# mazpie/genrl

Hardware: AMD Instinct MI355X
Metric: world-model+imag update steps/sec (B32xL32x64x64x3) (higher is better)
Workload: dtype f32 (storage, accumulation, every non-GEMM kernel and the fp32-MFMA GEMMs; the forward / dgrad / weight-gradient products of the imagination rollout, of the Dense+LN+SiLU chains from 192 rows up and of the encoder / decoder convolutions take fp32 operands pre-split into two fp16 planes of the scaled

## Files before the change

genrl_amd/csrc/dist.hip:

```cpp
#include "common.h"
#include <math.h>

namespace {

template <int W>
struct Cat {
  float p, pn, s;
  __device__ __forceinline__ void init(float logit, bool valid, int K, float a) {
    const float l = valid ? logit : -INFINITY;
    const float m = group_max<W>(l);
    const float e = valid ? expf(l - m) : 0.f;
    const float z = group_sum<W>(e);
    p = e / z;
    const float u = valid ? a * p + (1.0f - a) / K : 0.f;
    s = group_sum<W>(u);
    pn = u / s;
  }
  __device__ __forceinline__ float backward(float g, bool valid, float a) const {
    const float gi = valid ? g : 0.f;
    const float dot = group_sum<W>(gi * pn);
    const float du = (gi - dot) / s;
    const float dp = a * du;
    const float dot2 = group_sum<W>(valid ? dp * p : 0.f);
    return valid ? p * (dp - dot2) : 0.f;
// ... 119 lines not shown
  const float logit = sum + (bias ? bias[n0 + k] : 0.f);
  Cat<32> cat;
  cat.init(logit, valid, 32, a);
  const long g = (long)min(orow, M - 1) * S + lat;
  const float score = valid ? (q ? cat.pn / q[g * 32 + k] : cat.pn) : -INFINITY;
  const int best = group_argmax<32>(score, k);
  if (valid) {
    C[(long)orow * ldc + n0 + k] = logit;
    sample[g * 32 + k] = (k == best) ? 1.0f : 0.0f;
    const float sc2 = (sample2 || idx2) ? (scale2 ? scale2[orow] : 1.0f) : 1.0f;
    if (sample2) sample2[g * 32 + k] = (k == best) ? sc2 : 0.0f;
    if (idx2 && k == 0) idx2[g] = sc2 != 0.0f ? best : -1;
  }
}

template <int W>
__global__ __launch_bounds__(1024) void onehot_bwd_kernel(const float* __restrict__ logits,
                                                          const float* __restrict__ gsample,
                                                          float* __restrict__ dlogits, long G, int K, float a,
                                                          int accumulate, PlaneOut xo, int rowlen, MaskedGrad mg) {
  __shared__ float redm[16];
  const long g = ((long)blockIdx.x * blockDim.x + threadIdx.x) / W;
  const int k = threadIdx.x % W;
  const bool valid = (g < G) && (k < K);
  const long gi = g < G ? g : G - 1;
  const float l = valid ? logits[gi * K + k] : 0.f;
  Cat<W> c;
  c.init(l, valid, K, a);
  float gs = (valid && gsample) ? gsample[gi * K + k] : 0.f;
  if (valid && mg.g2) gs += (mg.scale ? mg.scale[gi / mg.S] : 1.0f) * mg.g2[gi * K + k];
  const float d = c.backward(gs, valid, a);
  float o = 0.f;
  if (valid) {
    o = accumulate ? dlogits[gi * K + k] + d : d;
    if (dlogits) dlogits[gi * K + k] = o;
  }
  if (xo.p) {
    const float am = wave_max(fabsf(o));
    if ((threadIdx.x & 63) == 0) redm[threadIdx.x >> 6] = am;
    __syncthreads();
    float m = redm[0];
    for (int w = 1; w < (int)(blockDim.x >> 6); ++w) m = fmaxf(m, redm[w]);
    const float inv = h2_inv_of(m);
    if (valid) h2_store1(xo, (long)blockIdx.x * xo.ld + threadIdx.x, o, h2_scale_of(inv));
    if (threadIdx.x == 0) xo.inv[blockIdx.x] = inv;
  }
}

template <int W>
__global__ __launch_bounds__(256) void cat_kl_fwd_kernel(const float* __restrict__ lp, const float* __restrict__ lq,
                                                         float* __restrict__ kl, float* __restrict__ ent_p,
                                                         float* __restrict__ ent_q, int S, int K, float a) {
  __shared__ float red[16];
  const long row = blockIdx.x;
  constexpr int GPB = 256 / W;
  const int k = threadIdx.x % W, gsub = threadIdx.x / W;
  float akl = 0.f, aep = 0.f, aeq = 0.f;
  for (int s0 = 0; s0 < S; s0 += GPB) {
    const int s = s0 + gsub;
// ... 35 lines not shown
  const float lpp = clamp_log(cp.pn), lqq = clamp_log(cq.pn);
  if (dlp) {
    const float d = cp.backward(valid ? (lpp - lqq + 1.0f) : 0.f, valid, a);
    if (valid) dlp[gi * K + k] = gp[row] * d;
  }
  if (dlq) {
    const float d = cq.backward(valid ? (-cp.pn / cq.pn) : 0.f, valid, a);
    if (valid) dlq[gi * K + k] = gq[row] * d;
  }
}

struct TwoHot {
  int below, above;
  float wb, wa;
};
__device__ __forceinline__ TwoHot twohot_target(const float* __restrict__ buckets, float x, int lane) {
  const float xs = symlogf_(x);
  int le = 0, gt = 0;
  for (int j = lane; j < 255; j += 64) {
    le += (buckets[j] <= xs);
    gt += (buckets[j] > xs);
  }
  le = (int)wave_sum((float)le);
  gt = (int)wave_sum((float)gt);
  TwoHot t;
  t.below = min(max(le - 1, 0), 254);
  t.above = min(max(255 - gt, 0), 254);
  const bool eq = t.below == t.above;
  const float db = eq ? 1.0f : fabsf(buckets[t.below] - xs);
  const float da = eq ? 1.0f : fabsf(buckets[t.above] - xs);
  const float tot = db + da;
  t.wb = da / tot;
  t.wa = db / tot;
  return t;
}

__global__ __launch_bounds__(256) void twohot_fwd_kernel(const float* __restrict__ logits,
                                                         const float* __restrict__ x,
                                                         const float* __restrict__ buckets, float* __restrict__ out,
                                                         long R, int mode, long ld) {
  const int lane = threadIdx.x & 63;
  const long row = (long)blockIdx.x * 4 + (threadIdx.x >> 6);
  if (row >= R) return;
  const float* lr = logits + row * ld;
  float m = -INFINITY;
  for (int j = lane; j < 255; j += 64) m = fmaxf(m, lr[j]);
  m = wave_max(m);
  float z = 0.f, sb = 0.f;
  for (int j = lane; j < 255; j += 64) {
    const float e = expf(lr[j] - m);
    z += e;
    sb += e * buckets[j];
  }
  z = wave_sum(z);
  if (mode == 1) {
    sb = wave_sum(sb);
    if (lane == 0) out[row] = symexpf_(sb / z);
    return;
  }
  const float lse = m + logf(z);
  const TwoHot t = twohot_target(buckets, x[row], lane);
  if (lane == 0) out[row] = t.wb * (lr[t.below] - lse) + t.wa * (lr[t.above] - lse);
}

__global__ __launch_bounds__(256) void twohot_bwd_kernel(const float* __restrict__ logits,
                                                         const float* __restrict__ x,
                                                         const float* __restrict__ buckets,
                                                         const float* __restrict__ gout, float* __restrict__ dlogits,
                                                         long R, int mode, long ld, long ldd) {
  const int lane = threadIdx.x & 63;
  const long row = (long)blockIdx.x * 4 + (threadIdx.x >> 6);
  if (row >= R) return;
  const float* lr = logits + row * ld;
  float m = -INFINITY;
  for (int j = lane; j < 255; j += 64) m = fmaxf(m, lr[j]);
  m = wave_max(m);
  float z = 0.f, sb = 0.f;
  for (int j = lane; j < 255; j += 64) {
    const float e = expf(lr[j] - m);
    z += e;
    sb += e * buckets[j];
  }
  z = wave_sum(z);
  sb = wave_sum(sb);
  const float g = gout[row];
  float* dr = dlogits + row * ldd;
  if (ldd > 255 && lane == 63) dr[255] = 0.f;
  if (mode == 1) {
    const float mu = sb / z;
    const float ds = g * expf(fabsf(mu));
    for (int j = lane; j < 255; j += 64) dr[j] = ds * (expf(lr[j] - m) / z) * (buckets[j] - mu);
    return;
  }
  const TwoHot t = twohot_target(buckets, x[row], lane);
  for (int j = lane; j < 255; j += 64) {
    float tg = 0.f;
    if (j == t.below) tg += t.wb;
    if (j == t.above) tg += t.wa;
    dr[j] = g * (tg - expf(lr[j] - m) / z);
  }
}

__global__ __launch_bounds__(256) void kl_balance_fwd_kernel(const float* __restrict__ kl, long R, float mix, float free_,
                                                            float* __restrict__ loss) {
  __shared__ float red[8];
  float a = 0.f;
  for (long i = threadIdx.x; i < R; i += 256) a += fmaxf(kl[i], free_);
  a = block_sum_256(a, red);
  if (threadIdx.x == 0) {
    const float m = a / (float)R;
    *loss = mix * m + (1.0f - mix) * m;
  }
}
__global__ void kl_balance_bwd_kernel(const float* __restrict__ kl, const float* __restrict__ gloss, long R, float mix,
// ... 42 lines not shown
  for (int i = threadIdx.x; i < E; i += 256) {
    const float d = mp[i] - ((float)op[i] / 255.0f - 0.5f);
    a += d * d;
  }
  a = block_sum_256(a, red);
  if (threadIdx.x == 0) like[n] = -a;
}
__global__ void mse_bwd_kernel(const float* __restrict__ mean, const uint8_t* __restrict__ obs,
                               const float* __restrict__ glike, float* __restrict__ dmean, long total, int E) {
  const long i = (long)blockIdx.x * blockDim.x + threadIdx.x;
  if (i >= total) return;
  const float d = mean[i] - ((float)obs[i] / 255.0f - 0.5f);
  dmean[i] = -2.0f * d * glike[i / E];
}

__global__ __launch_bounds__(256) void maxcos_fwd_kernel(const float* __restrict__ u, const float* __restrict__ v,
                                                         const long* __restrict__ urow, float* __restrict__ out,
                                                         long R, int E) {
  const int lane = threadIdx.x & 63;
  const long row = (long)blockIdx.x * 4 + (threadIdx.x >> 6);
  if (row >= R) return;
  const float* ur = u + (urow ? urow[row] : row) * E;
  const float* vr = v + row * E;
  float su = 0.f, sv = 0.f;
  for (int j = lane; j < E; j += 64) {
    su += ur[j] * ur[j];
    sv += vr[j] * vr[j];
  }
  const float mn = fmaxf(sqrtf(wave_sum(su)), sqrtf(wave_sum(sv)));
  float d = 0.f;
  for (int j = lane; j < E; j += 64) d += (ur[j] / mn) * (vr[j] / mn);
  d = wave_sum(d);
  if (lane == 0) out[row] = d;
}
__global__ __launch_bounds__(256) void maxcos_bwd_kernel(const float* __restrict__ u, const float* __restrict__ v,
                                                         const long* __restrict__ urow, const float* __restrict__ gout,
                                                         float* __restrict__ dv, long R, int E) {
  const int lane = threadIdx.x & 63;
  const long row = (long)blockIdx.x * 4 + (threadIdx.x >> 6);
  if (row >= R) return;
  const float* ur = u + (urow ? urow[row] : row) * E;
  const float* vr = v + row * E;
  float su = 0.f, sv = 0.f, uv = 0.f;
  for (int j = lane; j < E; j += 64) {
    su += ur[j] * ur[j];
    sv += vr[j] * vr[j];
    uv += ur[j] * vr[j];
  }
  su = wave_sum(su);
  sv = wave_sum(sv);
  uv = wave_sum(uv);
  const float g = gout[row];
  float* dr = dv + row * E;
  const float wv = sv > su ? 1.0f : (sv == su ? 0.5f : 0.0f);
  for (int j = lane; j < E; j += 64) dr[j] = g * (ur[j] / fmaxf(su, sv) - wv * 2.0f * uv * vr[j] / (sv * sv));
}

constexpr int AL_MAX_T = 32, AL_MAX_NF = 8, AL_MAX_D = AL_MAX_NF * (AL_MAX_T - AL_MAX_NF);
template <int EPT>
__global__ __launch_bounds__(256) void align_index_kernel(const float* __restrict__ ct, const float* __restrict__ ca,
                                                          long* __restrict__ urow, int T, long N, int E, int nf) {
  constexpr int AL_SLOTS = AL_MAX_D + AL_MAX_T + AL_MAX_NF;
  __shared__ float swave[4][AL_SLOTS];
  __shared__ float sdot[AL_SLOTS];
  __shared__ int sbest;
  const long n = blockIdx.x;
  const int W = T - nf;
  const int nd = nf * W, ntot = nd + T + nf;
  const int wv = threadIdx.x >> 6;
  const int lane = threadIdx.x & 63;
  float cj[AL_MAX_NF][EPT > 0 ? EPT : 1];
  if (EPT > 0) {
#pragma unroll
    for (int j = 0; j < AL_MAX_NF; ++j)
#pragma unroll
      for (int i = 0; i < EPT; ++i) {
        const int e = threadIdx.x + i * 256;
        cj[j][i] = (j < nf && e < E) ? ct[((long)j * N + n) * E + e] : 0.f;
      }
  }
  for (int tau = 0; tau < T; ++tau) {
    const float* vr = ca + ((long)tau * N + n) * E;
    float vv = 0.f;
    float d[AL_MAX_NF];
#pragma unroll
    for (int j = 0; j < AL_MAX_NF; ++j) d[j] = 0.f;
    if (EPT > 0) {
#pragma unroll
      for (int i = 0; i < EPT; ++i) {
        const int e = threadIdx.x + i * 256;
        const float v = e < E ? vr[e] : 0.f;
        vv += v * v;
#pragma unroll
        for (int j = 0; j < AL_MAX_NF; ++j) d[j] += v * cj[j][i];
      }
    } else {
      for (int e = threadIdx.x; e < E; e += 256) {
        const float v = vr[e];
        vv += v * v;
#pragma unroll
        for (int j = 0; j < AL_MAX_NF; ++j)
          if (j < nf) d[j] += v * ct[((long)j * N + n) * E + e];
      }
    }
    vv = wave_sum(vv);
    if (lane == 0) swave[wv][nd + tau] = vv;
#pragma unroll
    for (int j = 0; j < AL_MAX_NF; ++j) {
      if (j < nf) {
        const int t = tau - j;
        const float s = wave_sum(d[j]);
        if (lane == 0 && t >= 0 && t < W) swave[wv][t * nf + j] = s;
      }
    }
  }
  for (int j = 0; j < nf; ++j) {
    const float* ur = ct + ((long)j * N + n) * E;
    float uu = 0.f;
    if (EPT > 0) {
#pragma unroll
      for (int i = 0; i < EPT; ++i) {
        float c = 0.f;
#pragma unroll
        for (int jj = 0; jj < AL_MAX_NF; ++jj)
          if (jj == j) c = cj[jj][i];
        uu += c * c;
      }
// ... 64 lines not shown
int genrl_onehot_bwd_planes_only_ok(int K, int rowlen) {
  return (K == 4 || K == 8 || K == 16 || K == 32 || K == 64) && rowlen > 0 && rowlen % 64 == 0 && rowlen <= 1024 && rowlen % K == 0;
}

static int onehot_bwd_impl(const float* logits, const float* gsample, float* dlogits, long G, int K, float unimix,
                     int accumulate, PlaneOut xo, int rowlen, void* stream, MaskedGrad mg = MaskedGrad{nullptr, nullptr, 1}) {
  GENRL_ENTER();
  if (G <= 0) return GENRL_OK;
  if ((!gsample && !mg.g2) || (mg.g2 && mg.S <= 0)) return GENRL_EINVAL;
  if (xo.p && (rowlen <= 0 || xo.ld < rowlen || !xo.inv || rowlen % K || (G * K) % rowlen)) return GENRL_EINVAL;
  if (K > MAX_K) return GENRL_EINVAL;
  return dispatch_w(K, [&](auto w) {
    constexpr int W = decltype(w)::value;
    const bool rowblk = xo.p && genrl_onehot_bwd_planes_only_ok(K, rowlen);
    if (!dlogits && (accumulate || !rowblk)) return (int)GENRL_EINVAL;
    if (rowblk)
      hipLaunchKernelGGL((onehot_bwd_kernel<W>), dim3((G * K) / rowlen), dim3(rowlen), 0, (hipStream_t)stream, logits,
                         gsample, dlogits, G, K, unimix, accumulate, xo, rowlen, mg);
    else
      hipLaunchKernelGGL((onehot_bwd_kernel<W>), dim3(cdiv(G * W, 256)), dim3(256), 0, (hipStream_t)stream, logits,
                         gsample, dlogits, G, K, unimix, accumulate, PlaneOut{nullptr, 0, 0, nullptr}, rowlen, mg);
    GENRL_CHECK_LAUNCH();
    if (xo.p && !rowblk)
      return genrl_split_h2(dlogits, rowlen, (int)((G * K) / rowlen), rowlen, xo.p, xo.ld, xo.plane, xo.inv, 0, stream);
    return GENRL_OK;
  });
}
int genrl_onehot_bwd(const float* logits, const float* gsample, float* dlogits, long G, int K, float unimix,
                     int accumulate, void* stream) {
  return onehot_bwd_impl(logits, gsample, dlogits, G, K, unimix, accumulate, PlaneOut{nullptr, 0, 0, nullptr}, 1, stream);
}
int genrl_onehot_bwd_h2(const float* logits, const float* gsample, float* dlogits, long G, int K, float unimix,
                        int accumulate, uint16_t* dp, int rowlen, long ldp, long plane, float* inv, void* stream) {
  return onehot_bwd_impl(logits, gsample, dlogits, G, K, unimix, accumulate, PlaneOut{dp, ldp, plane, inv}, rowlen, stream);
}
// ... 73 lines not shown
  GENRL_CHECK_LAUNCH();
  return GENRL_OK;
}

int genrl_twohot_fwd(const float* logits, long ld, const float* x, const float* buckets, float* out, long R, int mode,
                     void* stream) {
  GENRL_ENTER();
  if (R <= 0) return GENRL_OK;
  if (ld < 255) return GENRL_EINVAL;
  hipLaunchKernelGGL(twohot_fwd_kernel, dim3(cdiv(R, 4)), dim3(256), 0, (hipStream_t)stream, logits, x, buckets, out, R,
                     mode, ld);
  GENRL_CHECK_LAUNCH();
  return GENRL_OK;
}

int genrl_twohot_bwd(const float* logits, long ld, const float* x, const float* buckets, const float* gout,
                     float* dlogits, long ldd, long R, int mode, void* stream) {
  GENRL_ENTER();
  if (R <= 0) return GENRL_OK;
  if (ld < 255 || ldd < 255) return GENRL_EINVAL;
  hipLaunchKernelGGL(twohot_bwd_kernel, dim3(cdiv(R, 4)), dim3(256), 0, (hipStream_t)stream, logits, x, buckets, gout,
                     dlogits, R, mode, ld, ldd);
  GENRL_CHECK_LAUNCH();
  return GENRL_OK;
}

int genrl_lambda_return_fwd(const float* reward, const float* value, float* ret, int H, long N, float disc, float lam,
                            void* stream) {
  GENRL_ENTER();
  if (N <= 0) return GENRL_OK;
  hipLaunchKernelGGL(lambda_return_fwd_kernel, dim3(cdiv(N, 256)), dim3(256), 0, (hipStream_t)stream, reward, value,
                     ret, H, N, disc, lam);
  GENRL_CHECK_LAUNCH();
  return GENRL_OK;
}

int genrl_lambda_return_bwd(const float* gret, float* dreward, float* dvalue, int H, long N, float disc, float lam,
                            int zero_tail, void* stream) {
  GENRL_ENTER();
// ... 14 lines not shown

int genrl_mse_bwd(const float* mean, const uint8_t* obs, const float* glike, float* dmean, long Nimg, int E,
                  void* stream) {
  GENRL_ENTER();
  const long total = Nimg * E;
  if (total <= 0) return GENRL_OK;
  hipLaunchKernelGGL(mse_bwd_kernel, dim3(cdiv(total, 256)), dim3(256), 0, (hipStream_t)stream, mean, obs, glike, dmean,
                     total, E);
  GENRL_CHECK_LAUNCH();
  return GENRL_OK;
}

int genrl_maxcos_fwd(const float* u, const float* v, const long* urow, float* out, long R, int E, void* stream) {
  GENRL_ENTER();
  if (R <= 0) return GENRL_OK;
  hipLaunchKernelGGL(maxcos_fwd_kernel, dim3(cdiv(R, 4)), dim3(256), 0, (hipStream_t)stream, u, v, urow, out, R, E);
  GENRL_CHECK_LAUNCH();
  return GENRL_OK;
}

int genrl_maxcos_bwd(const float* u, const float* v, const long* urow, const float* gout, float* dv, long R, int E,
                     void* stream) {
  GENRL_ENTER();
  if (R <= 0) return GENRL_OK;
  hipLaunchKernelGGL(maxcos_bwd_kernel, dim3(cdiv(R, 4)), dim3(256), 0, (hipStream_t)stream, u, v, urow, gout, dv, R,
                     E);
  GENRL_CHECK_LAUNCH();
  return GENRL_OK;
}

int genrl_align_index(const float* ct, const float* ca, long* urow, int T, long N, int E, int nf, void* stream) {
  GENRL_ENTER();
  if (N <= 0) return GENRL_OK;
  if (T > AL_MAX_T || nf > AL_MAX_NF || nf >= T) return GENRL_EINVAL;
#define GO(EPTV) hipLaunchKernelGGL((align_index_kernel<EPTV>), dim3(N), dim3(256), 0, (hipStream_t)stream, ct, ca, urow, T, N, E, nf)
  if (E <= 512) GO(2); else if (E <= 1024) GO(4); else if (E <= 1536) GO(6); else if (E <= 2048) GO(8); else GO(0);
#undef GO
  GENRL_CHECK_LAUNCH();
  return GENRL_OK;
}

// ... 2 lines not shown
```

genrl_amd/csrc/stats.hip:

```cpp
#include "actor_heads.h"
#include <algorithm>
#include <math.h>

namespace {

constexpr int NT = 1024;

__global__ __launch_bounds__(NT) void moments_kernel(const float* __restrict__ x, long n, float* __restrict__ out) {
  __shared__ double red[16];
  double s = 0.0, q = 0.0, a = 0.0;
  for (long i = threadIdx.x; i < n; i += NT) {
    const double v = x[i];
    s += v; q += v * v; a += fabs(v);
  }
  s = block_sum_d(s, red); q = block_sum_d(q, red); a = block_sum_d(a, red);
  if (threadIdx.x == 0) {
    const double mean = s / n;
    const double var = n > 1 ? fmax((q - n * mean * mean) / (n - 1), 0.0) : NAN;
    out[0] = (float)mean; out[1] = (float)sqrt(var); out[2] = (float)(a / n); out[3] = (float)(q / n);
  }
}

__device__ __forceinline__ unsigned key_of(float f) {
  const unsigned u = __builtin_bit_cast(unsigned, f);
  return (u & 0x80000000u) ? ~u : (u | 0x80000000u);
}
__device__ __forceinline__ float val_of(unsigned k) {
  const unsigned u = (k & 0x80000000u) ? (k & 0x7FFFFFFFu) : ~k;
  return __builtin_bit_cast(float, u);
}

__global__ __launch_bounds__(NT) void quantile_ema_kernel(const float* __restrict__ x, long n, float q0, float q1,
                                                           float alpha, float* __restrict__ ema,
                                                           float* __restrict__ out ) {
  __shared__ unsigned hist[4][256];
  __shared__ unsigned prefix[4];
  __shared__ long rank[4];
  __shared__ float wgt[2];
  __shared__ int slot[4], nslot;
  if (threadIdx.x == 0) {
    const float r0 = q0 * (float)(n - 1), r1 = q1 * (float)(n - 1);
    rank[0] = (long)floorf(r0); rank[1] = (long)ceilf(r0); rank[2] = (long)floorf(r1); rank[3] = (long)ceilf(r1);
    wgt[0] = r0 - floorf(r0); wgt[1] = r1 - floorf(r1);
    for (int s = 0; s < 4; ++s) prefix[s] = 0u;
  }
  constexpr int KPT = 16;
  const bool inreg = n <= (long)KPT * NT;
  unsigned keys[KPT];
  if (inreg) {
#pragma unroll
    for (int j = 0; j < KPT; ++j) {
      const long i = (long)j * NT + threadIdx.x;
      keys[j] = i < n ? key_of(x[i]) : 0u;
    }
  }
  for (int round = 0; round < 4; ++round) {
    const int shift = 24 - 8 * round;
    for (int i = threadIdx.x; i < 4 * 256; i += NT) (&hist[0][0])[i] = 0u;
    if (threadIdx.x == 0) {
      int ns = 0;
      for (int s2 = 0; s2 < 4; ++s2) {
        int found = -1;
        for (int t = 0; t < s2; ++t)
          if (prefix[t] == prefix[s2]) { found = slot[t]; break; }
        slot[s2] = found >= 0 ? found : ns++;
      }
      nslot = ns;
    }
    __syncthreads();
    const unsigned mask = round == 0 ? 0u : (0xFFFFFFFFu << (shift + 8));
    unsigned pf[4];
    const int ns = nslot;
#pragma unroll
    for (int h = 0; h < 4; ++h) pf[h] = 0xFFFFFFFFu;
#pragma unroll
    for (int s2 = 3; s2 >= 0; --s2) pf[slot[s2]] = prefix[s2];
    auto count = [&](unsigned k) {
#pragma unroll
      for (int h = 0; h < 4; ++h)
        if (h < ns && (k & mask) == pf[h]) atomicAdd(&hist[h][(k >> shift) & 255u], 1u);
    };
    if (inreg) {
#pragma unroll
      for (int j = 0; j < KPT; ++j)
        if ((long)j * NT + threadIdx.x < n) count(keys[j]);
    } else {
      for (long i = threadIdx.x; i < n; i += NT) count(key_of(x[i]));
    }
    __syncthreads();
    if (threadIdx.x < 4) {
      const int s2 = threadIdx.x, h = slot[s2];
      long r = rank[s2];
      int b = 0;
      for (; b < 255; ++b) {
        const unsigned c = hist[h][b];
        if (r < (long)c) break;
        r -= c;
      }
      rank[s2] = r;
      prefix[s2] |= ((unsigned)b) << shift;
    }
    __syncthreads();
  }
  if (threadIdx.x == 0) {
    const float v[4] = {val_of(prefix[0]), val_of(prefix[1]), val_of(prefix[2]), val_of(prefix[3])};
    float qv[2];
#pragma unroll
    for (int j = 0; j < 2; ++j) {
      const float a = v[2 * j], b = v[2 * j + 1], w = wgt[j];
      qv[j] = w < 0.5f ? a + w * (b - a) : b - (b - a) * (1.0f - w);
    }
    const float e0 = alpha * qv[0] + (1.0f - alpha) * ema[0], e1 = alpha * qv[1] + (1.0f - alpha) * ema[1];
    ema[0] = e0; ema[1] = e1;
    out[0] = e0; out[1] = fmaxf(e1 - e0, 1.0f); out[2] = qv[0]; out[3] = qv[1];
  }
// ... 231 lines not shown
```

genrl_amd/ops.py:

```python
import os
import ctypes
import torch
from torch.autograd import Function

from ._lib import lib, check, GenrlHipError, struct as _cstruct

UNIMIX = 0.99
gemm_profile = None


from .streams import raw_current_stream as _stream
from .streams import timed_start, timed_end


def _p(t):
    if t is None:
        return None
    if not t.is_cuda:
        raise GenrlHipError('genrl_amd ops need tensors on the MI355X (no CPU fallback)')
    assert t.is_contiguous(), 'non-contiguous tensor handed to a HIP op'
    return t.data_ptr()


_PREF = _cstruct('genrl_planes_ref')
# ... 519 lines not shown
        v = t.reshape(R, 255).contiguous()
    return v, (v.stride(0) if R > 1 else 255)


class _TwoHot(Function):
    @staticmethod
    def forward(ctx, logits, x, mode):
        lg, ld = _rows255(_f32(logits))
        R = lg.shape[0]
        b = twohot_buckets(lg.device)
        xx = x.reshape(R).contiguous() if x is not None else None
        out = torch.empty(R, device=lg.device)
        check(lib().genrl_twohot_fwd(_prows(lg), ld, _p(xx), _p(b), _p(out), R, mode, _stream()), 'twohot_fwd')
        ctx.save_for_backward(lg, xx if xx is not None else lg.new_empty(0))
        ctx.mode, ctx.ld, ctx.lshape = mode, ld, logits.shape
        return out.reshape(logits.shape[:-1])

    @staticmethod
    def backward(ctx, g):
        lg, xx = ctx.saved_tensors
        R = lg.shape[0]
        d = torch.empty(R, 256, device=lg.device)
        check(lib().genrl_twohot_bwd(_prows(lg), ctx.ld, _p(xx) if ctx.mode == 0 else None, _p(twohot_buckets(lg.device)),
                                     _p(g.reshape(R).contiguous()), _p(d), 256, R, ctx.mode, _stream()), 'twohot_bwd')
        return d[:, :255].view(ctx.lshape), None, None


def twohot_logprob(logits, x):
    return _TwoHot.apply(logits, x.detach(), 0)


def twohot_mean(logits):
    return _TwoHot.apply(logits, None, 1).unsqueeze(-1)



class _LambdaReturn(Function):
    @staticmethod
    def forward(ctx, reward, value, disc, lam):
        Hv = value.shape[0]
# ... 1912 lines not shown
```

genrl_amd/ops_planes.py:

```python
import os

import torch
from torch.autograd import Function

from ._lib import lib, check, struct as _cstruct
from . import planes
from . import planes as pl
from . import ops
from .ops import _p, _f32, _ln_param_targets, _wgrad_target, _bias_grad, sgemm, fill, UNIMIX

_stream = ops._stream


def _ln_fwd(pre_ptr, gamma, beta, y_ptr, mean_ptr, rstd_ptr, M, N, eps, P, row0):
    check(lib().genrl_ln_act_fwd_h2(pre_ptr, N, _p(gamma), _p(beta), y_ptr, N, mean_ptr, rstd_ptr, M, N, eps, 1,
                                    P.ptr(row0), P.ld, P.plane, P.inv_ptr(row0), _stream()), 'ln_act_fwd_h2')


def _ln_bwd(dy_ptr, pre_ptr, gamma, beta, mean_ptr, rstd_ptr, dpre_ptr, M, N, P, row0, g0=None, g1=None, g2=None, ws=None,
            acc_p=0):
    check(lib().genrl_ln_act_bwd_h2(dy_ptr, N, pre_ptr, N, _p(gamma), _p(beta), mean_ptr, rstd_ptr, dpre_ptr, N, _p(g0),
                                    _p(g1), _p(g2), _p(ws), M, N, 1, acc_p, P.ptr(row0), P.ld, P.plane, P.inv_ptr(row0),
                                    _stream()), 'ln_act_bwd_h2')

# ... 308 lines not shown
class _LinearPlanes(Function):
    @staticmethod
    def forward(ctx, x, W, b, P, r0):
        x2 = _f32(x).reshape(-1, x.shape[-1]).contiguous()
        M, K = x2.shape
        N = W.shape[0]
        if P is None:
            P, r0 = planes.split(x2), 0
        Np = (N + 3) // 4 * 4
        y = torch.empty(M, Np, device=x.device)
        planes.gemm(P, planes.weight(W), y, Np, b, M, N, a_row0=r0)
        ctx.save_for_backward(x2, W)
        ctx.bias = b
        ctx.xshape = x.shape
        ctx.in_planes = (P, r0) if (ctx.needs_input_grad[1] and planes.tn_ok(M, N, K, K) and r0 % 4 == 0) else None
        return (y if Np == N else y[:, :N]).view(*x.shape[:-1], N)

    @staticmethod
    def backward(ctx, dy):
        x2, W = ctx.saved_tensors
        M, K = x2.shape
        N = W.shape[0]
        b = ctx.bias
        dy2, ldy = ops._rows_ld(dy.reshape(M, N))
        dx = dW = db = None
        tn = ctx.needs_input_grad[1] and ctx.in_planes is not None and planes.tn_ok(M, N, K, K)
        dyp = planes.split(dy2) if (ctx.needs_input_grad[0] or tn) else None
        if ctx.needs_input_grad[0]:
            dx = torch.empty(M, K, device=dy.device)
            planes.gemm(dyp, planes.weight(W, transpose=True), dx, K, None, M, K)
            dx = dx.reshape(ctx.xshape)
        if ctx.needs_input_grad[1]:
            tgt, acc, dW = _wgrad_target(W)
            if tn:
                planes.gemm_tn(dyp, ctx.in_planes[0], tgt, K, N, K, M, accumulate=acc, b_row0=ctx.in_planes[1])
            else:
                sgemm(dy2, 1, ldy, x2, 1, K, tgt, K, None, N, K, M, accumulate=acc)
        if b is not None and ctx.needs_input_grad[2]:
            db = _bias_grad(b, dy2, ldy)
        return dx, dW, db, None, None


# ... 428 lines not shown
```

include/genrl_hip.h:

```cpp
#ifndef GENRL_HIP_H
#define GENRL_HIP_H
#include <stdint.h>
#ifdef __cplusplus
extern "C" {
#endif

long genrl_sgemm_ws_floats(int M, int N, int K);
int genrl_set_gemm_precision(int mode);
int genrl_sgemm_last_pipe(void);
int genrl_gemm_precision(void);
int genrl_sgemm(const float* A, long a_rs, long a_ks, const float* B, long b_rs, long b_ks, float* C, long ldc,
                const float* bias, int M, int N, int K, int accumulate, float* ws, long ws_floats, void* stream);

int genrl_sgemm_conv(const float* A, long a_rs, long a_ks, const float* B, long b_rs, long b_ks, float* C, long ldc,
                     const float* bias, int M, int N, int K, int accumulate, float* ws, long ws_floats, int which,
                     int img_h, int img_w, int img_c, int ksize, void* stream);

int genrl_split_h2(const float* x, long ldx, int R, int Cn, uint16_t* out, long ld_out, long plane, float* inv, int transpose,
                   void* stream);
int genrl_gemm_h2(const uint16_t* a0, long a0_ld, long a0_plane, const float* a0_inv, const uint16_t* b0, long b0_ld, long b0_plane,
                  const float* b0_inv, int k0, const uint16_t* a1, long a1_ld, long a1_plane, const float* a1_inv,
                  const uint16_t* b1, long b1_ld, long b1_plane, const float* b1_inv, int k1,
                  float* C, long ldc, const float* bias, int M, int N, int accumulate, void* stream);
int genrl_gemm_h2_pair(const uint16_t* a, long a_ld, long a_plane, const float* a_inv, int k,
// ... 245 lines not shown
int genrl_onehot_bwd_masked(const float* logits, const float* gsample, const float* g2, const float* scale2, int S, float* dlogits,
                            long G, int K, float unimix, int accumulate, void* stream);
int genrl_cat_kl_fwd(const float* lp, const float* lq, float* kl, float* ent_p, float* ent_q, long R, int S, int K,
                     float unimix, void* stream);
int genrl_cat_kl_bwd(const float* lp, const float* lq, const float* gp, const float* gq, float* dlp, float* dlq, long R,
                     int S, int K, float unimix, void* stream);

int genrl_kl_balance_fwd(const float* kl, long R, float mix, float free_nats, float* loss, void* stream);
int genrl_kl_balance_bwd(const float* kl, const float* gloss, long R, float mix, float free_nats, float* gp, float* gq,
                         void* stream);

int genrl_twohot_fwd(const float* logits, long ld, const float* x, const float* buckets, float* out, long R, int mode,
                     void* stream);
int genrl_twohot_bwd(const float* logits, long ld, const float* x, const float* buckets, const float* gout,
                     float* dlogits, long ldd, long R, int mode, void* stream);

int genrl_lambda_return_fwd(const float* reward, const float* value, float* ret, int H, long N, float disc, float lam,
                            void* stream);
int genrl_lambda_return_bwd(const float* gret, float* dreward, float* dvalue, int H, long N, float disc, float lam,
                            int zero_tail, void* stream);

int genrl_mse_fwd(const float* mean, const uint8_t* obs, float* like, long Nimg, int E, void* stream);
int genrl_mse_bwd(const float* mean, const uint8_t* obs, const float* glike, float* dmean, long Nimg, int E,
                  void* stream);

int genrl_maxcos_fwd(const float* u, const float* v, const long* urow, float* out, long R, int E, void* stream);
int genrl_maxcos_bwd(const float* u, const float* v, const long* urow, const float* gout, float* dv, long R, int E,
                     void* stream);
int genrl_align_index(const float* ct, const float* ca, long* urow, int T, long N, int E, int nf, void* stream);

// ... 93 lines not shown
```

Before: 48.21.

## Register-cache row kernels, fuse twohot grad plane split, ballot-based quantile histogram

Several small-kernel changes land together. The twohot backward now also writes the fp16 plane split of its gradient, and the downstream Dense layer reuses those planes instead of running its own split pass. The onehot backward uses 256-thread blocks that each handle several elements. Twohot, maxcos and align kernels keep row values in registers and use ballot/popcount or butterfly shuffles instead of repeated loads and reductions, and align prefetches the next timestep. The quantile EMA kernel aggregates histogram atomics per wave and finds the rank bin with a parallel prefix scan instead of a serial single-thread scan. Together these cut launches, global reloads and atomic contention, at the cost of more code and extra Python bookkeeping to match the handed-off planes.

```diff
diff --git a/genrl_amd/csrc/dist.hip b/genrl_amd/csrc/dist.hip
--- a/genrl_amd/csrc/dist.hip
+++ b/genrl_amd/csrc/dist.hip
@@ -157,35 +157,57 @@
   }
 }
 
-template <int W>
-__global__ __launch_bounds__(1024) void onehot_bwd_kernel(const float* __restrict__ logits,
-                                                          const float* __restrict__ gsample,
-                                                          float* __restrict__ dlogits, long G, int K, float a,
-                                                          int accumulate, PlaneOut xo, int rowlen, MaskedGrad mg) {
-  __shared__ float redm[16];
-  const long g = ((long)blockIdx.x * blockDim.x + threadIdx.x) / W;
+template <int W, int NI>
+__global__ __launch_bounds__(256) void onehot_bwd_kernel(const float* __restrict__ logits,
+                                                         const float* __restrict__ gsample,
+                                                         float* __restrict__ dlogits, long G, int K, float a,
+                                                         int accumulate, PlaneOut xo, int rowlen, MaskedGrad mg) {
+  __shared__ float redm[4];
+  const bool rows = xo.p != nullptr;
   const int k = threadIdx.x % W;
-  const bool valid = (g < G) && (k < K);
-  const long gi = g < G ? g : G - 1;
-  const float l = valid ? logits[gi * K + k] : 0.f;
-  Cat<W> c;
-  c.init(l, valid, K, a);
-  float gs = (valid && gsample) ? gsample[gi * K + k] : 0.f;
-  if (valid && mg.g2) gs += (mg.scale ? mg.scale[gi / mg.S] : 1.0f) * mg.g2[gi * K + k];
-  const float d = c.backward(gs, valid, a);
-  float o = 0.f;
-  if (valid) {
-    o = accumulate ? dlogits[gi * K + k] + d : d;
-    if (dlogits) dlogits[gi * K + k] = o;
-  }
-  if (xo.p) {
-    const float am = wave_max(fabsf(o));
+  const long base = rows ? (long)blockIdx.x * rowlen : (long)blockIdx.x * blockDim.x;
+  bool valid[NI];
+  long at[NI];
+  float l[NI], gs[NI], prev[NI], o[NI];
+#pragma unroll
+  for (int i = 0; i < NI; ++i) {
+    const int e = threadIdx.x + i * blockDim.x;
+    const long g = (base + e) / W;
+    valid[i] = (!rows || e < rowlen) && (g < G) && (k < K);
+    at[i] = (g < G ? g : G - 1) * K + k;
+    l[i] = valid[i] ? logits[at[i]] : 0.f;
+    gs[i] = (valid[i] && gsample) ? gsample[at[i]] : 0.f;
+    if (valid[i] && mg.g2) gs[i] += (mg.scale ? mg.scale[at[i] / K / mg.S] : 1.0f) * mg.g2[at[i]];
+    prev[i] = (valid[i] && accumulate) ? dlogits[at[i]] : 0.f;
+  }
+  float am = 0.f;
+#pragma unroll
+  for (int i = 0; i < NI; ++i) {
+    Cat<W> c;
+    c.init(l[i], valid[i], K, a);
+    const float d = c.backward(gs[i], valid[i], a);
+    o[i] = 0.f;
+    if (valid[i]) {
+      {
+#pragma clang fp contract(off)
+        o[i] = accumulate ? prev[i] + d : d;
+      }
+      if (dlogits) dlogits[at[i]] = o[i];
+    }
+    am = i == 0 ? fabsf(o[i]) : fmaxf(am, fabsf(o[i]));
+  }
+  if (rows) {
+    am = wave_max(am);
     if ((threadIdx.x & 63) == 0) redm[threadIdx.x >> 6] = am;
     __syncthreads();
     float m = redm[0];
     for (int w = 1; w < (int)(blockDim.x >> 6); ++w) m = fmaxf(m, redm[w]);
-    const float inv = h2_inv_of(m);
-    if (valid) h2_store1(xo, (long)blockIdx.x * xo.ld + threadIdx.x, o, h2_scale_of(inv));
+    const float inv = h2_inv_of(m), sc = h2_scale_of(inv);
+#pragma unroll
+    for (int i = 0; i < NI; ++i) {
+      const int e = threadIdx.x + i * blockDim.x;
+      if (e < rowlen) h2_store1(xo, (long)blockIdx.x * xo.ld + e, o[i], sc);
+    }
     if (threadIdx.x == 0) xo.inv[blockIdx.x] = inv;
   }
 }
@@ -251,15 +273,15 @@
   int below, above;
   float wb, wa;
 };
-__device__ __forceinline__ TwoHot twohot_target(const float* __restrict__ buckets, float x, int lane) {
+__device__ __forceinline__ TwoHot twohot_target(const float* __restrict__ buckets, const float (&b)[4], float x, int lane) {
   const float xs = symlogf_(x);
   int le = 0, gt = 0;
-  for (int j = lane; j < 255; j += 64) {
-    le += (buckets[j] <= xs);
-    gt += (buckets[j] > xs);
-  }
-  le = (int)wave_sum((float)le);
-  gt = (int)wave_sum((float)gt);
+#pragma unroll
+  for (int i = 0; i < 4; ++i) {
+    const bool in = lane + 64 * i < 255;
+    le += __popcll(__ballot(in && b[i] <= xs));
+    gt += __popcll(__ballot(in && b[i] > xs));
+  }
   TwoHot t;
   t.below = min(max(le - 1, 0), 254);
   t.above = min(max(255 - gt, 0), 254);
@@ -272,6 +294,38 @@
   return t;
 }
 
+struct TwoHotRow {
+  float l[4], b[4], e[4];
+  float m, z, sb;
+  __device__ __forceinline__ void load(const float* __restrict__ lr, const float* __restrict__ buckets, int lane) {
+#pragma unroll
+    for (int i = 0; i < 4; ++i) {
+      const int j = lane + 64 * i;
+      l[i] = j < 255 ? lr[j] : 0.f;
+      b[i] = j < 255 ? buckets[j] : 0.f;
+    }
+    m = -INFINITY;
+#pragma unroll
+    for (int i = 0; i < 4; ++i)
+      if (lane + 64 * i < 255) m = fmaxf(m, l[i]);
+    m = wave_max(m);
+    z = 0.f; sb = 0.f;
+#pragma unroll
+    for (int i = 0; i < 4; ++i) {
+      e[i] = 0.f;
+      if (lane + 64 * i < 255) {
+        e[i] = expf(l[i] - m);
+        z += e[i];
+        {
+#pragma clang fp contract(off)
+          sb = sb + e[i] * b[i];
+        }
+      }
+    }
+    z = wave_sum(z);
+  }
+};
+
 __global__ __launch_bounds__(256) void twohot_fwd_kernel(const float* __restrict__ logits,
                                                          const float* __restrict__ x,
                                                          const float* __restrict__ buckets, float* __restrict__ out,
@@ -280,23 +334,15 @@
   const long row = (long)blockIdx.x * 4 + (threadIdx.x >> 6);
   if (row >= R) return;
   const float* lr = logits + row * ld;
-  float m = -INFINITY;
-  for (int j = lane; j < 255; j += 64) m = fmaxf(m, lr[j]);
-  m = wave_max(m);
-  float z = 0.f, sb = 0.f;
-  for (int j = lane; j < 255; j += 64) {
-    const float e = expf(lr[j] - m);
-    z += e;
-    sb += e * buckets[j];
-  }
-  z = wave_sum(z);
+  TwoHotRow r;
+  r.load(lr, buckets, lane);
   if (mode == 1) {
-    sb = wave_sum(sb);
-    if (lane == 0) out[row] = symexpf_(sb / z);
+    const float sb = wave_sum(r.sb);
+    if (lane == 0) out[row] = symexpf_(sb / r.z);
     return;
   }
-  const float lse = m + logf(z);
-  const TwoHot t = twohot_target(buckets, x[row], lane);
+  const float lse = r.m + logf(r.z);
+  const TwoHot t = twohot_target(buckets, r.b, x[row], lane);
   if (lane == 0) out[row] = t.wb * (lr[t.below] - lse) + t.wa * (lr[t.above] - lse);
 }
 
@@ -304,37 +350,46 @@
                                                          const float* __restrict__ x,
                                                          const float* __restrict__ buckets,
                                                          const float* __restrict__ gout, float* __restrict__ dlogits,
-                                                         long R, int mode, long ld, long ldd) {
+                                                         long R, int mode, long ld, long ldd, PlaneOut xo) {
   const int lane = threadIdx.x & 63;
   const long row = (long)blockIdx.x * 4 + (threadIdx.x >> 6);
   if (row >= R) return;
-  const float* lr = logits + row * ld;
-  float m = -INFINITY;
-  for (int j = lane; j < 255; j += 64) m = fmaxf(m, lr[j]);
-  m = wave_max(m);
-  float z = 0.f, sb = 0.f;
-  for (int j = lane; j < 255; j += 64) {
-    const float e = expf(lr[j] - m);
-    z += e;
-    sb += e * buckets[j];
-  }
-  z = wave_sum(z);
-  sb = wave_sum(sb);
+  TwoHotRow r;
+  r.load(logits + row * ld, buckets, lane);
+  const float z = r.z, sb = wave_sum(r.sb);
   const float g = gout[row];
   float* dr = dlogits + row * ldd;
   if (ldd > 255 && lane == 63) dr[255] = 0.f;
+  float d[4] = {0.f, 0.f, 0.f, 0.f};
   if (mode == 1) {
     const float mu = sb / z;
     const float ds = g * expf(fabsf(mu));
-    for (int j = lane; j < 255; j += 64) dr[j] = ds * (expf(lr[j] - m) / z) * (buckets[j] - mu);
-    return;
-  }
-  const TwoHot t = twohot_target(buckets, x[row], lane);
-  for (int j = lane; j < 255; j += 64) {
-    float tg = 0.f;
-    if (j == t.below) tg += t.wb;
-    if (j == t.above) tg += t.wa;
-    dr[j] = g * (tg - expf(lr[j] - m) / z);
+#pragma unroll
+    for (int i = 0; i < 4; ++i)
+      if (lane + 64 * i < 255) d[i] = ds * (r.e[i] / z) * (r.b[i] - mu);
+  } else {
+    const TwoHot t = twohot_target(buckets, r.b, x[row], lane);
+#pragma unroll
+    for (int i = 0; i < 4; ++i) {
+      const int j = lane + 64 * i;
+      float tg = 0.f;
+      if (j == t.below) tg += t.wb;
+      if (j == t.above) tg += t.wa;
+      if (j < 255) d[i] = g * (tg - r.e[i] / z);
+    }
+  }
+#pragma unroll
+  for (int i = 0; i < 4; ++i)
+    if (lane + 64 * i < 255) dr[lane + 64 * i] = d[i];
+  if (xo.p) {
+    float am = 0.f;
+#pragma unroll
+    for (int i = 0; i < 4; ++i) am = fmaxf(am, fabsf(d[i]));
+    const float inv = h2_inv_of(wave_max(am)), sc = h2_scale_of(inv);
+    if (lane == 0) xo.inv[row] = inv;
+#pragma unroll
+    for (int i = 0; i < 4; ++i) h2_store1(xo, row * xo.ld + lane + 64 * i, d[i], sc);
+    for (long c = 256 + lane; c < xo.ld; c += 64) h2_store1(xo, row * xo.ld + c, 0.f, sc);
   }
 }
 
@@ -407,6 +462,19 @@
   dmean[i] = -2.0f * d * glike[i / E];
 }
 
+template <int NPL>
+struct MaxcosRows {
+  float u[NPL > 0 ? NPL : 1], v[NPL > 0 ? NPL : 1];
+  __device__ __forceinline__ void load(const float* __restrict__ ur, const float* __restrict__ vr, int lane, int E) {
+#pragma unroll
+    for (int i = 0; i < NPL; ++i) {
+      const int j = lane + 64 * i;
+      u[i] = j < E ? ur[j] : 0.f;
+      v[i] = j < E ? vr[j] : 0.f;
+    }
+  }
+};
+template <int NPL>
 __global__ __launch_bounds__(256) void maxcos_fwd_kernel(const float* __restrict__ u, const float* __restrict__ v,
                                                          const long* __restrict__ urow, float* __restrict__ out,
                                                          long R, int E) {
@@ -415,17 +483,32 @@
   if (row >= R) return;
   const float* ur = u + (urow ? urow[row] : row) * E;
   const float* vr = v + row * E;
-  float su = 0.f, sv = 0.f;
-  for (int j = lane; j < E; j += 64) {
-    su += ur[j] * ur[j];
-    sv += vr[j] * vr[j];
-  }
-  const float mn = fmaxf(sqrtf(wave_sum(su)), sqrtf(wave_sum(sv)));
-  float d = 0.f;
-  for (int j = lane; j < E; j += 64) d += (ur[j] / mn) * (vr[j] / mn);
+  float su = 0.f, sv = 0.f, d = 0.f;
+  if (NPL > 0) {
+    MaxcosRows<NPL> r;
+    r.load(ur, vr, lane, E);
+#pragma unroll
+    for (int i = 0; i < NPL; ++i)
+      if (lane + 64 * i < E) {
+        su += r.u[i] * r.u[i];
+        sv += r.v[i] * r.v[i];
+      }
+    const float mn = fmaxf(sqrtf(wave_sum(su)), sqrtf(wave_sum(sv)));
+#pragma unroll
+    for (int i = 0; i < NPL; ++i)
+      if (lane + 64 * i < E) d += (r.u[i] / mn) * (r.v[i] / mn);
+  } else {
+    for (int j = lane; j < E; j += 64) {
+      su += ur[j] * ur[j];
+      sv += vr[j] * vr[j];
+    }
+    const float mn = fmaxf(sqrtf(wave_sum(su)), sqrtf(wave_sum(sv)));
+    for (int j = lane; j < E; j += 64) d += (ur[j] / mn) * (vr[j] / mn);
+  }
   d = wave_sum(d);
   if (lane == 0) out[row] = d;
 }
+template <int NPL>
 __global__ __launch_bounds__(256) void maxcos_bwd_kernel(const float* __restrict__ u, const float* __restrict__ v,
                                                          const long* __restrict__ urow, const float* __restrict__ gout,
                                                          float* __restrict__ dv, long R, int E) {
@@ -434,11 +517,23 @@
   if (row >= R) return;
   const float* ur = u + (urow ? urow[row] : row) * E;
   const float* vr = v + row * E;
+  MaxcosRows<NPL> r;
+  r.load(ur, vr, lane, E);
   float su = 0.f, sv = 0.f, uv = 0.f;
-  for (int j = lane; j < E; j += 64) {
-    su += ur[j] * ur[j];
-    sv += vr[j] * vr[j];
-    uv += ur[j] * vr[j];
+  if (NPL > 0) {
+#pragma unroll
+    for (int i = 0; i < NPL; ++i)
+      if (lane + 64 * i < E) {
+        su += r.u[i] * r.u[i];
+        sv += r.v[i] * r.v[i];
+        uv += r.u[i] * r.v[i];
+      }
+  } else {
+    for (int j = lane; j < E; j += 64) {
+      su += ur[j] * ur[j];
+      sv += vr[j] * vr[j];
+      uv += ur[j] * vr[j];
+    }
   }
   su = wave_sum(su);
   sv = wave_sum(sv);
@@ -446,7 +541,13 @@
   const float g = gout[row];
   float* dr = dv + row * E;
   const float wv = sv > su ? 1.0f : (sv == su ? 0.5f : 0.0f);
-  for (int j = lane; j < E; j += 64) dr[j] = g * (ur[j] / fmaxf(su, sv) - wv * 2.0f * uv * vr[j] / (sv * sv));
+  if (NPL > 0) {
+#pragma unroll
+    for (int i = 0; i < NPL; ++i)
+      if (lane + 64 * i < E) dr[lane + 64 * i] = g * (r.u[i] / fmaxf(su, sv) - wv * 2.0f * uv * r.v[i] / (sv * sv));
+  } else {
+    for (int j = lane; j < E; j += 64) dr[j] = g * (ur[j] / fmaxf(su, sv) - wv * 2.0f * uv * vr[j] / (sv * sv));
+  }
 }
 
 constexpr int AL_MAX_T = 32, AL_MAX_NF = 8, AL_MAX_D = AL_MAX_NF * (AL_MAX_T - AL_MAX_NF);
@@ -472,6 +573,14 @@
         cj[j][i] = (j < nf && e < E) ? ct[((long)j * N + n) * E + e] : 0.f;
       }
   }
+  float vn[EPT > 0 ? EPT : 1];
+  if (EPT > 0) {
+#pragma unroll
+    for (int i = 0; i < EPT; ++i) {
+      const int e = threadIdx.x + i * 256;
+      vn[i] = e < E ? ca[n * E + e] : 0.f;
+    }
+  }
   for (int tau = 0; tau < T; ++tau) {
     const float* vr = ca + ((long)tau * N + n) * E;
     float vv = 0.f;
@@ -479,10 +588,20 @@
 #pragma unroll
     for (int j = 0; j < AL_MAX_NF; ++j) d[j] = 0.f;
     if (EPT > 0) {
+      float vc[EPT > 0 ? EPT : 1];
+#pragma unroll
+      for (int i = 0; i < EPT; ++i) vc[i] = vn[i];
+      if (tau + 1 < T) {
+        const float* vr1 = ca + ((long)(tau + 1) * N + n) * E;
+#pragma unroll
+        for (int i = 0; i < EPT; ++i) {
+          const int e = threadIdx.x + i * 256;
+          vn[i] = e < E ? vr1[e] : 0.f;
+        }
+      }
 #pragma unroll
       for (int i = 0; i < EPT; ++i) {
-        const int e = threadIdx.x + i * 256;
-        const float v = e < E ? vr[e] : 0.f;
+        const float v = vc[i];
         vv += v * v;
 #pragma unroll
         for (int j = 0; j < AL_MAX_NF; ++j) d[j] += v * cj[j][i];
@@ -496,14 +615,18 @@
           if (j < nf) d[j] += v * ct[((long)j * N + n) * E + e];
       }
     }
-    vv = wave_sum(vv);
-    if (lane == 0) swave[wv][nd + tau] = vv;
-#pragma unroll
-    for (int j = 0; j < AL_MAX_NF; ++j) {
-      if (j < nf) {
+#pragma unroll
+    for (int o = 32; o > 0; o >>= 1) {
+      vv += __shfl_xor(vv, o, 64);
+#pragma unroll
+      for (int j = 0; j < AL_MAX_NF; ++j) d[j] += __shfl_xor(d[j], o, 64);
+    }
+    if (lane == 0) {
+      swave[wv][nd + tau] = vv;
+#pragma unroll
+      for (int j = 0; j < AL_MAX_NF; ++j) {
         const int t = tau - j;
-        const float s = wave_sum(d[j]);
-        if (lane == 0 && t >= 0 && t < W) swave[wv][t * nf + j] = s;
+        if (j < nf && t >= 0 && t < W) swave[wv][t * nf + j] = d[j];
       }
     }
   }
@@ -598,11 +721,14 @@
     constexpr int W = decltype(w)::value;
     const bool rowblk = xo.p && genrl_onehot_bwd_planes_only_ok(K, rowlen);
     if (!dlogits && (accumulate || !rowblk)) return (int)GENRL_EINVAL;
-    if (rowblk)
-      hipLaunchKernelGGL((onehot_bwd_kernel<W>), dim3((G * K) / rowlen), dim3(rowlen), 0, (hipStream_t)stream, logits,
-                         gsample, dlogits, G, K, unimix, accumulate, xo, rowlen, mg);
+    if (rowblk && rowlen > 256)
+      hipLaunchKernelGGL((onehot_bwd_kernel<W, 4>), dim3((G * K) / rowlen), dim3(256), 0, (hipStream_t)stream, logits, gsample, dlogits, G, K,
+                         unimix, accumulate, xo, rowlen, mg);
+    else if (rowblk)
+      hipLaunchKernelGGL((onehot_bwd_kernel<W, 1>), dim3((G * K) / rowlen), dim3(rowlen), 0, (hipStream_t)stream, logits, gsample, dlogits, G,
+                         K, unimix, accumulate, xo, rowlen, mg);
     else
-      hipLaunchKernelGGL((onehot_bwd_kernel<W>), dim3(cdiv(G * W, 256)), dim3(256), 0, (hipStream_t)stream, logits,
+      hipLaunchKernelGGL((onehot_bwd_kernel<W, 1>), dim3(cdiv(G * W, 256)), dim3(256), 0, (hipStream_t)stream, logits,
                          gsample, dlogits, G, K, unimix, accumulate, PlaneOut{nullptr, 0, 0, nullptr}, rowlen, mg);
     GENRL_CHECK_LAUNCH();
     if (xo.p && !rowblk)
@@ -706,15 +832,25 @@
   return GENRL_OK;
 }
 
+static int twohot_bwd_impl(const float* logits, long ld, const float* x, const float* buckets, const float* gout, float* dlogits,
+                           long ldd, long R, int mode, PlaneOut xo, void* stream) {
+  GENRL_ENTER();
+  if (R <= 0) return GENRL_OK;
+  if (ld < 255 || ldd < 255) return GENRL_EINVAL;
+  if (xo.p && (xo.ld < 256 || (xo.ld & 63) || !xo.inv)) return GENRL_EINVAL;
+  hipLaunchKernelGGL(twohot_bwd_kernel, dim3(cdiv(R, 4)), dim3(256), 0, (hipStream_t)stream, logits, x, buckets, gout,
+                     dlogits, R, mode, ld, ldd, xo);
+  GENRL_CHECK_LAUNCH();
+  return GENRL_OK;
+}
 int genrl_twohot_bwd(const float* logits, long ld, const float* x, const float* buckets, const float* gout,
                      float* dlogits, long ldd, long R, int mode, void* stream) {
-  GENRL_ENTER();
-  if (R <= 0) return GENRL_OK;
-  if (ld < 255 || ldd < 255) return GENRL_EINVAL;
-  hipLaunchKernelGGL(twohot_bwd_kernel, dim3(cdiv(R, 4)), dim3(256), 0, (hipStream_t)stream, logits, x, buckets, gout,
-                     dlogits, R, mode, ld, ldd);
-  GENRL_CHECK_LAUNCH();
-  return GENRL_OK;
+  return twohot_bwd_impl(logits, ld, x, buckets, gout, dlogits, ldd, R, mode, PlaneOut{nullptr, 0, 0, nullptr}, stream);
+}
+int genrl_twohot_bwd_h2(const float* logits, long ld, const float* x, const float* buckets, const float* gout,
+                        float* dlogits, long ldd, long R, int mode, uint16_t* dp, long ldp, long plane, float* inv, void* stream) {
+  if (!dp) return GENRL_EINVAL;
+  return twohot_bwd_impl(logits, ld, x, buckets, gout, dlogits, ldd, R, mode, PlaneOut{dp, ldp, plane, inv}, stream);
 }
 
 int genrl_lambda_return_fwd(const float* reward, const float* value, float* ret, int H, long N, float disc, float lam,
@@ -759,7 +895,9 @@
 int genrl_maxcos_fwd(const float* u, const float* v, const long* urow, float* out, long R, int E, void* stream) {
   GENRL_ENTER();
   if (R <= 0) return GENRL_OK;
-  hipLaunchKernelGGL(maxcos_fwd_kernel, dim3(cdiv(R, 4)), dim3(256), 0, (hipStream_t)stream, u, v, urow, out, R, E);
+#define GO(NPL) hipLaunchKernelGGL((maxcos_fwd_kernel<NPL>), dim3(cdiv(R, 4)), dim3(256), 0, (hipStream_t)stream, u, v, urow, out, R, E)
+  if (E <= 128) GO(2); else if (E <= 512) GO(8); else if (E <= 1536) GO(24); else GO(0);
+#undef GO
   GENRL_CHECK_LAUNCH();
   return GENRL_OK;
 }
@@ -768,8 +906,9 @@
                      void* stream) {
   GENRL_ENTER();
   if (R <= 0) return GENRL_OK;
-  hipLaunchKernelGGL(maxcos_bwd_kernel, dim3(cdiv(R, 4)), dim3(256), 0, (hipStream_t)stream, u, v, urow, gout, dv, R,
-                     E);
+#define GO(NPL) hipLaunchKernelGGL((maxcos_bwd_kernel<NPL>), dim3(cdiv(R, 4)), dim3(256), 0, (hipStream_t)stream, u, v, urow, gout, dv, R, E)
+  if (E <= 128) GO(2); else if (E <= 512) GO(8); else if (E <= 1536) GO(24); else GO(0);
+#undef GO
   GENRL_CHECK_LAUNCH();
   return GENRL_OK;
 }
diff --git a/genrl_amd/csrc/stats.hip b/genrl_amd/csrc/stats.hip
--- a/genrl_amd/csrc/stats.hip
+++ b/genrl_amd/csrc/stats.hip
@@ -30,6 +30,7 @@
   return __builtin_bit_cast(float, u);
 }
 
+constexpr int Q_PEEL = 2;
 __global__ __launch_bounds__(NT) void quantile_ema_kernel(const float* __restrict__ x, long n, float q0, float q1,
                                                            float alpha, float* __restrict__ ema,
                                                            float* __restrict__ out ) {
@@ -37,7 +38,7 @@
   __shared__ unsigned prefix[4];
   __shared__ long rank[4];
   __shared__ float wgt[2];
-  __shared__ int slot[4], nslot;
+  const int lane = threadIdx.x & 63;
   if (threadIdx.x == 0) {
     const float r0 = q0 * (float)(n - 1), r1 = q1 * (float)(n - 1);
     rank[0] = (long)floorf(r0); rank[1] = (long)ceilf(r0); rank[2] = (long)floorf(r1); rank[3] = (long)ceilf(r1);
@@ -57,48 +58,83 @@
   for (int round = 0; round < 4; ++round) {
     const int shift = 24 - 8 * round;
     for (int i = threadIdx.x; i < 4 * 256; i += NT) (&hist[0][0])[i] = 0u;
-    if (threadIdx.x == 0) {
-      int ns = 0;
-      for (int s2 = 0; s2 < 4; ++s2) {
-        int found = -1;
-        for (int t = 0; t < s2; ++t)
-          if (prefix[t] == prefix[s2]) { found = slot[t]; break; }
-        slot[s2] = found >= 0 ? found : ns++;
-      }
-      nslot = ns;
-    }
     __syncthreads();
+    unsigned pr[4];
+    int slot[4], ns = 0;
+#pragma unroll
+    for (int s2 = 0; s2 < 4; ++s2) pr[s2] = prefix[s2];
+#pragma unroll
+    for (int s2 = 0; s2 < 4; ++s2) {
+      int found = -1;
+#pragma unroll
+      for (int t = s2 - 1; t >= 0; --t)
+        if (pr[t] == pr[s2]) found = slot[t];
+      slot[s2] = found >= 0 ? found : ns++;
+    }
     const unsigned mask = round == 0 ? 0u : (0xFFFFFFFFu << (shift + 8));
     unsigned pf[4];
-    const int ns = nslot;
 #pragma unroll
     for (int h = 0; h < 4; ++h) pf[h] = 0xFFFFFFFFu;
 #pragma unroll
-    for (int s2 = 3; s2 >= 0; --s2) pf[slot[s2]] = prefix[s2];
-    auto count = [&](unsigned k) {
+    for (int s2 = 3; s2 >= 0; --s2) {
 #pragma unroll
       for (int h = 0; h < 4; ++h)
-        if (h < ns && (k & mask) == pf[h]) atomicAdd(&hist[h][(k >> shift) & 255u], 1u);
+        if (slot[s2] == h) pf[h] = pr[s2];
+    }
+    auto count = [&](bool have, unsigned k) {
+      int bin = -1;
+#pragma unroll
+      for (int h = 0; h < 4; ++h)
+        if (have && h < ns && (k & mask) == pf[h]) bin = h * 256 + (int)((k >> shift) & 255u);
+      bool todo = bin >= 0;
+#pragma unroll
+      for (int it = 0; it < Q_PEEL; ++it) {
+        const unsigned long long act = __ballot(todo);
+        if (act == 0ull) break;
+        const int leader = __ffsll((long long)act) - 1;
+        const int lb = __shfl(bin, leader, 64);
+        const bool same = todo && bin == lb;
+        const unsigned long long sm = __ballot(same);
+        if (lane == leader) atomicAdd(&(&hist[0][0])[lb], (unsigned)__popcll(sm));
+        todo = todo && !same;
+      }
+      if (todo) atomicAdd(&(&hist[0][0])[bin], 1u);
     };
     if (inreg) {
 #pragma unroll
-      for (int j = 0; j < KPT; ++j)
-        if ((long)j * NT + threadIdx.x < n) count(keys[j]);
+      for (int j = 0; j < KPT; ++j) count((long)j * NT + threadIdx.x < n, keys[j]);
     } else {
-      for (long i = threadIdx.x; i < n; i += NT) count(key_of(x[i]));
+      for (long i0 = 0; i0 < n; i0 += NT) {
+        const long i = i0 + threadIdx.x;
+        count(i < n, i < n ? key_of(x[i]) : 0u);
+      }
     }
     __syncthreads();
-    if (threadIdx.x < 4) {
-      const int s2 = threadIdx.x, h = slot[s2];
-      long r = rank[s2];
-      int b = 0;
-      for (; b < 255; ++b) {
-        const unsigned c = hist[h][b];
-        if (r < (long)c) break;
-        r -= c;
+    if (threadIdx.x < 4 * 64) {
+      const int s2 = threadIdx.x >> 6;
+      int h = 0;
+#pragma unroll
+      for (int t = 0; t < 4; ++t)
+        if (t == s2) h = slot[t];
+      const long r = rank[s2];
+      unsigned long long c[4], sum = 0ull;
+#pragma unroll
+      for (int q = 0; q < 4; ++q) { c[q] = hist[h][4 * lane + q]; sum += c[q]; }
+      unsigned long long inc = sum;
+#pragma unroll
+      for (int o = 1; o < 64; o <<= 1) {
+        const unsigned long long up = __shfl_up(inc, o, 64);
+        if (lane >= o) inc += up;
       }
-      rank[s2] = r;
-      prefix[s2] |= ((unsigned)b) << shift;
+      const unsigned long long ur = (unsigned long long)r, a0 = inc - sum + c[0], a1 = a0 + c[1], a2 = a1 + c[2];
+      const unsigned long long hit = __ballot(ur < inc);
+      const int fl = hit ? __ffsll((long long)hit) - 1 : 63;
+      if (lane == fl) {
+        const int q = ur < a0 ? 0 : ur < a1 ? 1 : ur < a2 ? 2 : 3;
+        const unsigned long long before = q == 0 ? inc - sum : q == 1 ? a0 : q == 2 ? a1 : a2;
+        rank[s2] = (long)(ur - before);
+        prefix[s2] |= ((unsigned)(4 * lane + q)) << shift;
+      }
     }
     __syncthreads();
   }
diff --git a/genrl_amd/ops.py b/genrl_amd/ops.py
--- a/genrl_amd/ops.py
+++ b/genrl_amd/ops.py
@@ -557,6 +557,8 @@
         check(lib().genrl_twohot_fwd(_prows(lg), ld, _p(xx), _p(b), _p(out), R, mode, _stream()), 'twohot_fwd')
         ctx.save_for_backward(lg, xx if xx is not None else lg.new_empty(0))
         ctx.mode, ctx.ld, ctx.lshape = mode, ld, logits.shape
+        fn = logits.grad_fn
+        ctx.dy_consumer = fn if getattr(fn, 'takes_dy_planes', False) else None
         return out.reshape(logits.shape[:-1])
 
     @staticmethod
@@ -564,9 +566,17 @@
         lg, xx = ctx.saved_tensors
         R = lg.shape[0]
         d = torch.empty(R, 256, device=lg.device)
-        check(lib().genrl_twohot_bwd(_prows(lg), ctx.ld, _p(xx) if ctx.mode == 0 else None, _p(twohot_buckets(lg.device)),
-                                     _p(g.reshape(R).contiguous()), _p(d), 256, R, ctx.mode, _stream()), 'twohot_bwd')
-        return d[:, :255].view(ctx.lshape), None, None
+        args = (_prows(lg), ctx.ld, _p(xx) if ctx.mode == 0 else None, _p(twohot_buckets(lg.device)), _p(g.reshape(R).contiguous()),
+                _p(d), 256, R, ctx.mode)
+        dv = d[:, :255].view(ctx.lshape)
+        if ctx.dy_consumer is not None:
+            from . import planes
+            P = planes.Planes(R, 255, lg.device, zero=False)
+            check(lib().genrl_twohot_bwd_h2(*args, P.ptr(), P.ld, P.plane, P.inv_ptr(), _stream()), 'twohot_bwd_h2')
+            ctx.dy_consumer.dy_planes = (dv, P)
+        else:
+            check(lib().genrl_twohot_bwd(*args, _stream()), 'twohot_bwd')
+        return dv, None, None
 
 
 def twohot_logprob(logits, x):
diff --git a/genrl_amd/ops_planes.py b/genrl_amd/ops_planes.py
--- a/genrl_amd/ops_planes.py
+++ b/genrl_amd/ops_planes.py
@@ -346,6 +346,7 @@
         ctx.bias = b
         ctx.xshape = x.shape
         ctx.in_planes = (P, r0) if (ctx.needs_input_grad[1] and planes.tn_ok(M, N, K, K) and r0 % 4 == 0) else None
+        ctx.takes_dy_planes = bool(ctx.needs_input_grad[0] or ctx.in_planes is not None)
         return (y if Np == N else y[:, :N]).view(*x.shape[:-1], N)
 
     @staticmethod
@@ -357,7 +358,14 @@
         dy2, ldy = ops._rows_ld(dy.reshape(M, N))
         dx = dW = db = None
         tn = ctx.needs_input_grad[1] and ctx.in_planes is not None and planes.tn_ok(M, N, K, K)
-        dyp = planes.split(dy2) if (ctx.needs_input_grad[0] or tn) else None
+        dyp = None
+        if ctx.needs_input_grad[0] or tn:
+            given, ctx.dy_planes = getattr(ctx, 'dy_planes', None), None
+            if (given is not None and given[0].data_ptr() == dy.data_ptr() and given[0].shape == dy.shape and given[0].stride() == dy.stride()
+                    and given[1].rows == M and given[1].cols == N):
+                dyp = given[1]
+            else:
+                dyp = planes.split(dy2)
         if ctx.needs_input_grad[0]:
             dx = torch.empty(M, K, device=dy.device)
             planes.gemm(dyp, planes.weight(W, transpose=True), dx, K, None, M, K)
diff --git a/include/genrl_hip.h b/include/genrl_hip.h
--- a/include/genrl_hip.h
+++ b/include/genrl_hip.h
@@ -283,6 +283,8 @@
                      void* stream);
 int genrl_twohot_bwd(const float* logits, long ld, const float* x, const float* buckets, const float* gout,
                      float* dlogits, long ldd, long R, int mode, void* stream);
+int genrl_twohot_bwd_h2(const float* logits, long ld, const float* x, const float* buckets, const float* gout,
+                        float* dlogits, long ldd, long R, int mode, uint16_t* dp, long ldp, long plane, float* inv, void* stream);
 
 int genrl_lambda_return_fwd(const float* reward, const float* value, float* ret, int H, long N, float disc, float lam,
                             void* stream);
```

Result: no change. 48.66 (median of 6 runs) (+0.9%).
